# mkeeter/fidget

Hardware: AMD Instinct MI355X
Metric: Mvoxel/s (interval+point eval) on prospero.vm 1024^3 (higher is better)
Workload: dtype f32; 1 GPU; prospero.vm 3D heightmap+normals 1024^3, HipShape render hints (the library's tiles: 128/32/8, or 32/8 when the root level has few tiles), world_to_model=I

## Files before the change

fidget_amd/csrc/prune2.hip:

```cpp
#pragma once
#include <hip/hip_runtime.h>

#include "render_state.h"

#define FH_P2_WPC 4
#define FH_P2_PER_SLOT ((64 + FH_P2_WPB - 1) / FH_P2_WPB)
enum { FH_LK_OUT = 0, FH_LK_NONE = 1, FH_LK_A = 2, FH_LK_RR = 3, FH_LK_COPY = 4, FH_LK_CRR = 5, FH_LK_CRI = 6 };
#define FH_LK_CHOICE 0x8000u
#define FH_LK_IMM 0x4000u

namespace fhp2 {
__device__ __forceinline__ uint32_t rfl(uint32_t v) { return __builtin_amdgcn_readfirstlane(v); }
__device__ __forceinline__ uint64_t rfl64(uint64_t v) { return (uint64_t)rfl((uint32_t)v) | ((uint64_t)rfl((uint32_t)(v >> 32)) << 32); }
__device__ __forceinline__ uint32_t excl_sum(uint32_t v, uint32_t lane, uint32_t& total) {
    uint32_t x = v;
#pragma unroll
    for (int d = 1; d < 64; d <<= 1) {
        const uint32_t y = __shfl_up(x, d, 64);
        if ((int)lane >= d) x += y;
    }
    total = __shfl(x, 63, 64);
    return x - v;
}
__device__ __forceinline__ void p2_scan_batch2(uint32_t u, uint32_t& rel, uint32_t& out, uint32_t& maxro, uint32_t cnt, uint32_t kabs0) {
#if defined(__HIP_DEVICE_COMPILE__)
    uint32_t k, su, ro, kabs = kabs0;
    asm volatile(
        "s_mov_b32 %[k], 0\n"
        "L_p2b_loop_%=:\n\t"
        "v_readlane_b32 %[su], %[u], %[k]\n\t"
        "v_cmp_ge_u32 vcc, %[kabs], %[rel]\n\t"
        "s_add_u32 %[kabs], %[kabs], 1\n\t"
        "s_nop 0\n\t"
        "s_ff1_i32_b64 %[ro], vcc\n\t"
        "s_mov_b32 m0, %[ro]\n\t"
        "s_max_u32 %[maxro], %[maxro], %[ro]\n\t"
        "s_nop 0\n\t"
        "v_writelane_b32 %[rel], %[su], m0\n\t"
        "s_mov_b32 m0, %[k]\n\t"
        "s_add_u32 %[k], %[k], 1\n\t"
        "v_writelane_b32 %[out], %[ro], m0\n\t"
        "s_cmp_lt_u32 %[k], %[cnt]\n\t"
        "s_cbranch_scc1 L_p2b_loop_%="
        : [rel] "+v"(rel), [out] "+v"(out), [maxro] "+s"(maxro), [kabs] "+s"(kabs), [k] "=&s"(k), [su] "=&s"(su), [ro] "=&s"(ro)
        : [u] "v"(u), [cnt] "s"(cnt)
        : "m0", "scc", "vcc", "memory");
#else
    (void)u; (void)rel; (void)out; (void)maxro; (void)cnt; (void)kabs0;
#endif
}
}

__device__ __forceinline__ void p2_item(FhRenderState* S, uint32_t level, uint32_t big, uint32_t cw_stride, const uint2* __restrict__ links,
                                        const uint2* __restrict__ ctab, uint32_t flags, uint32_t cap_ops, uint32_t cap_choices, uint32_t cap_kept,
                                        const uint32_t* __restrict__ chain, uint32_t n_chain, uint32_t blk, char* smem) {
    using namespace fhp2;
    constexpr uint32_t W = FH_P2_WPC;
    const uint32_t lane = threadIdx.x & 63, wave = rfl(threadIdx.x >> 6);
    const uint32_t wpb = FH_P2_WPB, per_slot = (64 + wpb - 1) / wpb;
    const uint32_t kid = wave / W, sub = wave % W, tid = sub * 64 + lane;
    const bool lead = sub == kid % W;
    const uint32_t sidx = blk / per_slot;
    const uint32_t G = rfl(S->n_tgroups);
    if (sidx * G >= rfl(S->n_slots[big][level])) return;
    FhSlot& sl = S->slots[big][(size_t)sidx * G];
    if (sl.act == 0) return;
    const uint32_t c0 = (blk % per_slot) * wpb, c = c0 + kid;
    {
        bool any = false;
        for (uint32_t k = 0; k < wpb; k++) any |= c0 + k < 64 && sl.c_len[c0 + k] == 0xFFFFFFFFu;
        if (!any) return;
    }
    const uint32_t off = rfl(sl.tape.off), n = rfl(sl.tape.len), nch = rfl((uint32_t)sl.tape.n_choices);
    if (n > cap_ops || nch > cap_choices) return;
    const uint2* const ops = (const uint2*)(S->arena + off);
    const uint2* const lks = links;
    uint32_t* const chl = (uint32_t*)(smem + (size_t)FH_P2_WPB * fh_p2_wave_lds(cap_choices, cap_kept));
    for (uint32_t i = threadIdx.x; i < n_chain; i += blockDim.x) chl[i] = chain[i];
    char* const mine = smem + (size_t)kid * fh_p2_wave_lds(cap_choices, cap_kept);
    uint64_t* const mask = (uint64_t*)mine;
    uint16_t* const pref = (uint16_t*)(mine + 1024);
    uint16_t* const E = (uint16_t*)(mine + 1280);
    uint2* const comp = (uint2*)(mine + 1280 + (((size_t)cap_choices * 2 + 15) & ~(size_t)15));
    uint32_t* const lastuse = (uint32_t*)((char*)comp + (size_t)cap_kept * 8);
    uint8_t* const regb = (uint8_t*)((char*)lastuse + (size_t)cap_kept * 4);
    uint32_t* const red = (uint32_t*)(regb + (size_t)cap_kept * 3);
    const uint32_t nw = (n + 63) >> 6;
    bool on = c < 64 && rfl(sl.c_len[min(c, 63u)]) == 0xFFFFFFFFu;
    if (on && tid < 4) red[tid] = 0;
    const uint32_t* const cws = S->chwr + (size_t)sidx * G * cw_stride * 64;
    uint32_t* const cwl = (uint32_t*)comp;
    if (on) for (uint32_t k = tid; k < (nch + 15) / 16; k += 64 * W) cwl[k] = cws[(size_t)k * 64 + c];
    __syncthreads();

    const bool probe = S->want_stats != 0 && (flags & 2u) != 0 && lead;
    const uint64_t t_a = probe ? clock64() : 0;
    if (on) {
        const uint32_t nb = (nch + 63) >> 6;
        uint2 tn = (sub * 64 + lane) < nch ? ctab[sub * 64 + lane] : make_uint2(0, 0);
        for (uint32_t bi = sub; bi < nb; bi += W) {
            const uint32_t q0 = bi << 6, q = q0 + lane;
            const uint2 t = tn;
            if (q + 64 * W < nch) tn = ctab[q + 64 * W];
            uint32_t e = 0;
            if (q < nch) {
                const uint32_t i = t.y & 0xFFFFu, kind = t.y >> 16;
                const uint32_t ch = (cwl[q >> 4] >> ((q & 15) * 2)) & 3u;
                if (ch == FH_CHOICE_LEFT) e = t.x & 0xFFFFu;
                else if (ch == FH_CHOICE_RIGHT) e = kind == FH_LK_CRR ? t.x >> 16 : (i | FH_LK_IMM);
                else e = i;
            }
            for (int round = 0; round < 6; round++) {
                const bool inside = (e & FH_LK_CHOICE) != 0 && (e & 0x7FFFu) >= q0;
                if (__ballot(inside) == 0) break;
                const uint32_t t2 = __shfl(e, (int)((e & 0x7FFFu) - q0) & 63, 64);
                if (inside) e = t2;
            }
            if (q < nch) E[q] = (uint16_t)e;
        }
    }
    __syncthreads();
    if (on && lead) {
        for (uint32_t q0 = 0; q0 < nch; q0 += 64) {
            const uint32_t q = q0 + lane;
            const uint32_t e = q < nch ? (uint32_t)E[q] : 0u;
            const bool ptr = (e & FH_LK_CHOICE) != 0;
            if (__ballot(ptr) == 0) continue;
            if (ptr) E[q] = E[e & 0x7FFFu];
        }
    }
    __syncthreads();
    auto resolve = [&](uint2 l, bool& has_a, bool& has_b, bool& imm, uint32_t& ta, uint32_t& tb) {
        const uint32_t kind = (l.x >> 8) & 0xFFu, fa = l.y & 0xFFFFu, fb = l.y >> 16;
        const uint32_t e_own = E[kind == FH_LK_CRI ? (l.x >> 16) : 0u];
        const uint32_t e_a = E[((fa & FH_LK_CHOICE) && fa != 0xFFFFu) ? (fa & 0x7FFFu) : 0u], e_b = E[((fb & FH_LK_CHOICE) && fb != 0xFFFFu) ? (fb & 0x7FFFu) : 0u];
        imm = kind == FH_LK_CRI && (e_own & FH_LK_IMM) != 0;
        has_a = !imm && kind != FH_LK_NONE;
        has_b = !imm && (kind == FH_LK_RR || kind == FH_LK_CRR);
        ta = (fa & FH_LK_CHOICE) ? (e_a & 0x3FFFu) : fa;
        tb = (fb & FH_LK_CHOICE) ? (e_b & 0x3FFFu) : fb;
    };

    const uint64_t t_b1 = probe ? clock64() : 0;
    if (on && lead) {
        for (uint32_t k = lane; k < 128; k += 64) mask[k] = (k == ((n - 1) >> 6)) ? 1ull << ((n - 1) & 63) : 0ull;
        const uint32_t cw_bytes = (((nch + 15) / 16) * 4 + 15) & ~15u;
        uint16_t* const queue = (uint16_t*)((char*)comp + cw_bytes);
        const uint32_t qcap = (cap_kept * 8u - cw_bytes) / 2u;
        if (lane == 0) queue[0] = (uint16_t)(n - 1);
        uint32_t head = 0, tail = 1;
        bool over = false;
        const uint64_t below = (1ull << lane) - 1;
        for (uint32_t top = n_chain; top > 0;) {
            const uint32_t cnt = min(64u, top);
            uint32_t ch = 0, i = 0;
            if (lane < cnt) {
                const uint32_t e = chl[top - 1 - lane], q = e & 0xFFFFu;
                i = e >> 16;
                ch = (cwl[q >> 4] >> ((q & 15) * 2)) & 3u;
            }
            const uint64_t cut = __ballot(ch == FH_CHOICE_RIGHT);
            const bool seed = ch == FH_CHOICE_BOTH && (cut == 0 || lane < (uint32_t)__builtin_ctzll(cut));
            if (seed) atomicOr((unsigned long long*)&mask[i >> 6], 1ull << (i & 63));
            const uint64_t ms = __ballot(seed);
            if (tail + (uint32_t)__popcll(ms) > qcap) { over = true; break; }
            if (seed) queue[tail + (uint32_t)__popcll(ms & below)] = (uint16_t)i;
            tail += (uint32_t)__popcll(ms);
            if (cut) break;
            top -= cnt;
        }
        while (!over && head < tail) {
            const uint32_t cnt = min(64u, tail - head);
            bool has_a = false, has_b = false, imm = false;
            uint32_t ta = 0, tb = 0;
            if (lane < cnt) resolve(lks[queue[head + lane]], has_a, has_b, imm, ta, tb);
            head += cnt;
            bool new_a = false, new_b = false;
            if (has_a) { const uint64_t bit = 1ull << (ta & 63); new_a = (atomicOr((unsigned long long*)&mask[ta >> 6], bit) & bit) == 0; }
            if (has_b) { const uint64_t bit = 1ull << (tb & 63); new_b = (atomicOr((unsigned long long*)&mask[tb >> 6], bit) & bit) == 0; }
            const uint64_t ma = __ballot(new_a), mb = __ballot(new_b);
            const uint32_t na = (uint32_t)__popcll(ma), nb = (uint32_t)__popcll(mb);
            if (tail + na + nb > qcap) { over = true; break; }
            if (new_a) queue[tail + (uint32_t)__popcll(ma & below)] = (uint16_t)ta;
            if (new_b) queue[tail + na + (uint32_t)__popcll(mb & below)] = (uint16_t)tb;
            tail += na + nb;
        }
        if (over && lane == 0) red[3] = 1;
    }
    if (on && lead) {
        const uint32_t k0 = lane < nw ? (uint32_t)__popcll(mask[lane]) : 0u, k1 = lane + 64 < nw ? (uint32_t)__popcll(mask[lane + 64]) : 0u;
        uint32_t t0, t1;
        const uint32_t e0 = excl_sum(k0, lane, t0), e1 = excl_sum(k1, lane, t1);
        pref[lane] = (uint16_t)e0; pref[lane + 64] = (uint16_t)(t0 + e1);
        if (lane == 0) { red[0] = t0 + t1; if (t0 + t1 > cap_kept) red[3] = 1; }
    }
    __syncthreads();
    const uint64_t t_b2 = probe ? clock64() : 0;
    const uint32_t m = on ? rfl(red[0]) : 0u;
    if (on && rfl(red[3]) != 0) {
        if (probe && lane == 0) atomicAdd(&S->leaf_stat[5], 1ull << 32);
        on = false;
    }
    if (on) for (uint32_t k = tid; k < m; k += 64 * W) lastuse[k] = 0;
    __syncthreads();
    auto pos_of = [&](uint32_t t) -> uint32_t { return (uint32_t)pref[t >> 6] + (uint32_t)__popcll(mask[t >> 6] & ((1ull << (t & 63)) - 1)); };
    if (on) {
        for (uint32_t b = sub; b < nw; b += W) {
            const uint64_t word = rfl64(mask[b]);
            if (word == 0) continue;
            if ((word >> lane) & 1) {
                const uint32_t i = (b << 6) | lane;
                const uint32_t p = (uint32_t)pref[b] + (uint32_t)__popcll(word & ((1ull << lane) - 1));
                const uint2 l = lks[i];
                bool has_a, has_b, imm;
                uint32_t ta, tb;
                resolve(l, has_a, has_b, imm, ta, tb);
                const uint32_t kind = (l.x >> 8) & 0xFFu;
                uint32_t pa = 0, pb = 0;
                if (has_a) { pa = pos_of(ta); atomicMax(&lastuse[pa], p); }
                if (has_b) { pb = pos_of(tb); atomicMax(&lastuse[pb], p); }
                const uint32_t fl = (has_a ? 1u : 0u) | (has_b ? 2u : 0u) | (imm ? 4u : 0u) | ((kind >= FH_LK_CRR && !imm) ? 8u : 0u) | (kind == FH_LK_OUT ? 16u : 0u);
                comp[p] = make_uint2(pa | (pb << 16), i | (fl << 16));
            }
        }
    }
    __syncthreads();
    const uint64_t t_b3 = probe ? clock64() : 0;
    if (on && lead) {
        uint32_t maxro = 0, rel = 0;
        for (uint32_t base = 0; base < m; base += 64) {
            const uint32_t pl = base + lane;
            const uint32_t u = pl < m ? lastuse[pl] : 0u;
            uint32_t outv = 0;
            p2_scan_batch2(u, rel, outv, maxro, min(64u, m - base), base);
            if (pl < m) regb[pl] = (uint8_t)outv;
        }
        if (maxro >= 64u) {
            if (probe && lane == 0) { atomicAdd(&S->leaf_stat[4], 1ull << 32); atomicMax(&S->leaf_stat[6], (unsigned long long)m << 32); }
            if (lane == 0) red[3] = 1;
        }
    }
    __syncthreads();
    if (on && rfl(red[3]) != 0) on = false;
    const uint32_t end = on ? rfl(sl.c_off[c]) : 0u;
    if (on) {
        uint64_t* const dst = S->arena + (end - m);
        uint32_t high = 0, kept = 0;
        for (uint32_t pl = tid; pl < m; pl += 64 * W) {
            const uint2 cr = comp[pl];
            const uint32_t fl = cr.y >> 16, i = cr.y & 0xFFFFu, pa = cr.x & 0xFFFFu, pb = cr.x >> 16;
            const uint2 opw = ops[i];
            const uint32_t ro = regb[pl], ra = (fl & 1u) ? regb[pa] : 0u, rb = (fl & 2u) ? regb[pb] : 0u;
            uint64_t word;
            if (fl & 4u) word = fh_pack(FH_COPY_IMM, ro, 0, 0, opw.y);
            else if (fl & 16u) word = fh_pack(FH_OUTPUT, 0, ra, 0, opw.y);
            else word = (uint64_t)((opw.x & 0xFFu) | (ro << 8) | (ra << 20)) | ((uint64_t)((fl & 2u) ? rb : opw.y) << 32);
            dst[pl] = word;
            high = max(high, (fl & 16u) ? 0u : ro + 1u);
            kept += (fl >> 3) & 1u;
        }
#pragma unroll
        for (int dlt = 32; dlt > 0; dlt >>= 1) { high = max(high, (uint32_t)__shfl_xor(high, dlt, 64)); kept += (uint32_t)__shfl_xor(kept, dlt, 64); }
        if (lane == 0) { atomicMax(&red[1], high); atomicAdd(&red[2], kept); }
    }
    __syncthreads();
    if (probe && on && lane == 0) {
        const uint64_t t_e = clock64();
        atomicMax(&S->leaf_stat[4], (unsigned long long)(t_b1 - t_a)); atomicMax(&S->leaf_stat[5], (unsigned long long)(t_b2 - t_b1));
        atomicMax(&S->leaf_stat[6], (unsigned long long)(t_b3 - t_b2)); atomicMax(&S->leaf_stat[7], (unsigned long long)(t_e - t_b3));
    }
    if (on && lead && lane == 0) { sl.c_off[c] = end - m; sl.c_len[c] = m; sl.c_rc[c] = red[1] | (red[2] << 16); }
}

__global__ void __launch_bounds__(FH_P2_WPB * FH_P2_WPC * 64) k_prune2(FhRenderState* S, uint32_t level, uint32_t big, uint32_t cw_stride, const uint2* __restrict__ links,
                                                const uint2* __restrict__ ctab, uint32_t flags, uint32_t cap_ops, uint32_t cap_choices, uint32_t cap_kept,
                                                const uint32_t* __restrict__ chain, uint32_t n_chain) {
    extern __shared__ __attribute__((aligned(16))) char smem[];
    p2_item(S, level, big, cw_stride, links, ctab, flags, cap_ops, cap_choices, cap_kept, chain, n_chain, blockIdx.x, smem);
}
```

Baseline: 9.328 million Mvoxel/s.

## Prefetch and batch loads across phases of the tape pruning kernel

Restructures the prune2 kernel to issue global loads earlier. Choice-table entries are loaded before the barrier, two blocks are processed per wave iteration, and the pointer-fix pass prefetches the next E entry. The link-compaction phase now iterates over the BFS queue with link words loaded into registers ahead of time. Ops and comp entries are fetched before the serial register-allocation scan so their latency overlaps it. The intent is to hide global-memory latency behind barriers and serial sections. In exchange it uses more registers and adds a new overflow cap based on FH_P2_B2_PER; the queue-order iteration also relies on the queue holding exactly the kept nodes.

```diff
diff --git a/fidget_amd/csrc/prune2.hip b/fidget_amd/csrc/prune2.hip
--- a/fidget_amd/csrc/prune2.hip
+++ b/fidget_amd/csrc/prune2.hip
@@ -4,6 +4,7 @@
 #include "render_state.h"
 
 #define FH_P2_WPC 4
+#define FH_P2_B2_PER ((FH_P2_MAX_KEPT + FH_P2_WPC * 64 - 1) / (FH_P2_WPC * 64))
 #define FH_P2_PER_SLOT ((64 + FH_P2_WPB - 1) / FH_P2_WPB)
 enum { FH_LK_OUT = 0, FH_LK_NONE = 1, FH_LK_A = 2, FH_LK_RR = 3, FH_LK_COPY = 4, FH_LK_CRR = 5, FH_LK_CRI = 6 };
 #define FH_LK_CHOICE 0x8000u
@@ -87,46 +88,50 @@
     uint32_t* const red = (uint32_t*)(regb + (size_t)cap_kept * 3);
     const uint32_t nw = (n + 63) >> 6;
     bool on = c < 64 && rfl(sl.c_len[min(c, 63u)]) == 0xFFFFFFFFu;
+    const uint32_t end_v = on ? sl.c_off[c] : 0u;
     if (on && tid < 4) red[tid] = 0;
     const uint32_t* const cws = S->chwr + (size_t)sidx * G * cw_stride * 64;
     uint32_t* const cwl = (uint32_t*)comp;
     if (on) for (uint32_t k = tid; k < (nch + 15) / 16; k += 64 * W) cwl[k] = cws[(size_t)k * 64 + c];
+    uint2 tn = (on && tid < nch) ? ctab[tid] : make_uint2(0, 0);
+    uint2 tn1 = (on && tid + 64 * W < nch) ? ctab[tid + 64 * W] : make_uint2(0, 0);
     __syncthreads();
 
     const bool probe = S->want_stats != 0 && (flags & 2u) != 0 && lead;
     const uint64_t t_a = probe ? clock64() : 0;
     if (on) {
         const uint32_t nb = (nch + 63) >> 6;
-        uint2 tn = (sub * 64 + lane) < nch ? ctab[sub * 64 + lane] : make_uint2(0, 0);
-        for (uint32_t bi = sub; bi < nb; bi += W) {
-            const uint32_t q0 = bi << 6, q = q0 + lane;
-            const uint2 t = tn;
-            if (q + 64 * W < nch) tn = ctab[q + 64 * W];
-            uint32_t e = 0;
-            if (q < nch) {
-                const uint32_t i = t.y & 0xFFFFu, kind = t.y >> 16;
-                const uint32_t ch = (cwl[q >> 4] >> ((q & 15) * 2)) & 3u;
-                if (ch == FH_CHOICE_LEFT) e = t.x & 0xFFFFu;
-                else if (ch == FH_CHOICE_RIGHT) e = kind == FH_LK_CRR ? t.x >> 16 : (i | FH_LK_IMM);
-                else e = i;
+        auto first = [&](uint2 t, uint32_t q) -> uint32_t {
+            const uint32_t i = t.y & 0xFFFFu, kind = t.y >> 16;
+            const uint32_t ch = (cwl[q >> 4] >> ((q & 15) * 2)) & 3u;
+            if (ch == FH_CHOICE_LEFT) return t.x & 0xFFFFu;
+            if (ch == FH_CHOICE_RIGHT) return kind == FH_LK_CRR ? t.x >> 16 : (i | FH_LK_IMM);
+            return i;
+        };
+        for (uint32_t bi = sub; bi < nb; bi += 2 * W) {
+            const uint32_t qa0 = bi << 6, qb0 = (bi + W) << 6, qa = qa0 + lane, qb = qb0 + lane;
+            const uint2 t0 = tn, t1 = tn1;
+            if (qa + 128 * W < nch) tn = ctab[qa + 128 * W];
+            if (qb + 128 * W < nch) tn1 = ctab[qb + 128 * W];
+            uint32_t ea = qa < nch ? first(t0, qa) : 0u, eb = qb < nch ? first(t1, qb) : 0u;
+            for (int round = 0; round < 6; round++) {
+                const bool ia = (ea & FH_LK_CHOICE) != 0 && (ea & 0x7FFFu) >= qa0, ib = (eb & FH_LK_CHOICE) != 0 && (eb & 0x7FFFu) >= qb0;
+                if (__ballot(ia || ib) == 0) break;
+                const uint32_t xa = __shfl(ea, (int)((ea & 0x7FFFu) - qa0) & 63, 64), xb = __shfl(eb, (int)((eb & 0x7FFFu) - qb0) & 63, 64);
+                if (ia) ea = xa;
+                if (ib) eb = xb;
             }
-            for (int round = 0; round < 6; round++) {
-                const bool inside = (e & FH_LK_CHOICE) != 0 && (e & 0x7FFFu) >= q0;
-                if (__ballot(inside) == 0) break;
-                const uint32_t t2 = __shfl(e, (int)((e & 0x7FFFu) - q0) & 63, 64);
-                if (inside) e = t2;
-            }
-            if (q < nch) E[q] = (uint16_t)e;
+            if (qa < nch) E[qa] = (uint16_t)ea;
+            if (qb < nch) E[qb] = (uint16_t)eb;
         }
     }
     __syncthreads();
     if (on && lead) {
+        uint32_t en = lane < nch ? (uint32_t)E[lane] : 0u;
         for (uint32_t q0 = 0; q0 < nch; q0 += 64) {
-            const uint32_t q = q0 + lane;
-            const uint32_t e = q < nch ? (uint32_t)E[q] : 0u;
-            const bool ptr = (e & FH_LK_CHOICE) != 0;
-            if (__ballot(ptr) == 0) continue;
-            if (ptr) E[q] = E[e & 0x7FFFu];
+            const uint32_t q = q0 + lane, e = en;
+            if (q0 + 64 < nch) en = q + 64 < nch ? (uint32_t)E[q + 64] : 0u;
+            if (e & FH_LK_CHOICE) E[q] = E[e & 0x7FFFu];
         }
     }
     __syncthreads();
@@ -141,12 +146,12 @@
         tb = (fb & FH_LK_CHOICE) ? (e_b & 0x3FFFu) : fb;
     };
 
+    const uint32_t cw_bytes = (((nch + 15) / 16) * 4 + 15) & ~15u;
+    uint16_t* const queue = (uint16_t*)((char*)comp + cw_bytes);
+    const uint32_t qcap = (cap_kept * 8u - cw_bytes) / 2u;
     const uint64_t t_b1 = probe ? clock64() : 0;
     if (on && lead) {
         for (uint32_t k = lane; k < 128; k += 64) mask[k] = (k == ((n - 1) >> 6)) ? 1ull << ((n - 1) & 63) : 0ull;
-        const uint32_t cw_bytes = (((nch + 15) / 16) * 4 + 15) & ~15u;
-        uint16_t* const queue = (uint16_t*)((char*)comp + cw_bytes);
-        const uint32_t qcap = (cap_kept * 8u - cw_bytes) / 2u;
         if (lane == 0) queue[0] = (uint16_t)(n - 1);
         uint32_t head = 0, tail = 1;
         bool over = false;
@@ -192,7 +197,7 @@
         uint32_t t0, t1;
         const uint32_t e0 = excl_sum(k0, lane, t0), e1 = excl_sum(k1, lane, t1);
         pref[lane] = (uint16_t)e0; pref[lane + 64] = (uint16_t)(t0 + e1);
-        if (lane == 0) { red[0] = t0 + t1; if (t0 + t1 > cap_kept) red[3] = 1; }
+        if (lane == 0) { red[0] = t0 + t1; if (t0 + t1 > min(cap_kept, FH_P2_B2_PER * 64u * W)) red[3] = 1; }
     }
     __syncthreads();
     const uint64_t t_b2 = probe ? clock64() : 0;
@@ -201,17 +206,27 @@
         if (probe && lane == 0) atomicAdd(&S->leaf_stat[5], 1ull << 32);
         on = false;
     }
-    if (on) for (uint32_t k = tid; k < m; k += 64 * W) lastuse[k] = 0;
+    uint32_t qi[FH_P2_B2_PER];
+    uint2 ql[FH_P2_B2_PER];
+    if (on) {
+#pragma unroll
+        for (uint32_t r = 0; r < FH_P2_B2_PER; r++) {
+            const uint32_t k = tid + r * 64 * W;
+            if (r * 64 * W < m) {
+                qi[r] = k < m ? min((uint32_t)queue[k], n - 1) : n - 1;
+                ql[r] = lks[qi[r]];
+            }
+        }
+        for (uint32_t k = tid; k < m; k += 64 * W) lastuse[k] = 0;
+    }
     __syncthreads();
     auto pos_of = [&](uint32_t t) -> uint32_t { return (uint32_t)pref[t >> 6] + (uint32_t)__popcll(mask[t >> 6] & ((1ull << (t & 63)) - 1)); };
     if (on) {
-        for (uint32_t b = sub; b < nw; b += W) {
-            const uint64_t word = rfl64(mask[b]);
-            if (word == 0) continue;
-            if ((word >> lane) & 1) {
-                const uint32_t i = (b << 6) | lane;
-                const uint32_t p = (uint32_t)pref[b] + (uint32_t)__popcll(word & ((1ull << lane) - 1));
-                const uint2 l = lks[i];
+#pragma unroll
+        for (uint32_t r = 0; r < FH_P2_B2_PER; r++) {
+            if (tid + r * 64 * W < m) {
+                const uint32_t i = qi[r], p = pos_of(i);
+                const uint2 l = ql[r];
                 bool has_a, has_b, imm;
                 uint32_t ta, tb;
                 resolve(l, has_a, has_b, imm, ta, tb);
@@ -226,6 +241,12 @@
     }
     __syncthreads();
     const uint64_t t_b3 = probe ? clock64() : 0;
+    uint2 pc[FH_P2_B2_PER], po[FH_P2_B2_PER];
+    if (on) {
+#pragma unroll
+        for (uint32_t r = 0; r < FH_P2_B2_PER; r++)
+            if (tid + r * 64 * W < m) { pc[r] = comp[tid + r * 64 * W]; po[r] = ops[pc[r].y & 0xFFFFu]; }
+    }
     if (on && lead) {
         uint32_t maxro = 0, rel = 0;
         for (uint32_t base = 0; base < m; base += 64) {
@@ -242,14 +263,16 @@
     }
     __syncthreads();
     if (on && rfl(red[3]) != 0) on = false;
-    const uint32_t end = on ? rfl(sl.c_off[c]) : 0u;
+    const uint32_t end = on ? rfl(end_v) : 0u;
     if (on) {
         uint64_t* const dst = S->arena + (end - m);
         uint32_t high = 0, kept = 0;
-        for (uint32_t pl = tid; pl < m; pl += 64 * W) {
-            const uint2 cr = comp[pl];
-            const uint32_t fl = cr.y >> 16, i = cr.y & 0xFFFFu, pa = cr.x & 0xFFFFu, pb = cr.x >> 16;
-            const uint2 opw = ops[i];
+#pragma unroll
+        for (uint32_t r = 0; r < FH_P2_B2_PER; r++) {
+            const uint32_t pl = tid + r * 64 * W;
+            if (pl >= m) break;
+            const uint2 cr = pc[r], opw = po[r];
+            const uint32_t fl = cr.y >> 16, pa = cr.x & 0xFFFFu, pb = cr.x >> 16;
             const uint32_t ro = regb[pl], ra = (fl & 1u) ? regb[pa] : 0u, rb = (fl & 2u) ? regb[pb] : 0u;
             uint64_t word;
             if (fl & 4u) word = fh_pack(FH_COPY_IMM, ro, 0, 0, opw.y);
```

Result: slower. 9.154 million Mvoxel/s (-1.9%).
